# bmerry/mlsgpu

Measured on AMD Instinct MI355X. Metric: Mvoxels/s evaluated+triangulated, higher is better.
Workload: dtype f32; 1 GPU; cfg3: 512^3 grid, 50000000 splats (uniform), 27 buckets of <= 171 cells per side, octree+MLS+MC end-to-end; bucket_splats_total=52997386, mesh_memory_mb=4096, device_workers=3, batch=8, marching_group=2, mls_variant=culled+matrix-prefilter, counts_cover=the whole cloud

## Files before the change

mlsgpu_amd/csrc/api.hip:

```cpp
#include "common.hpp"

#include <algorithm>
#include <atomic>
#include <mutex>

using namespace mlsgpu;

namespace mlsgpu
{

static thread_local char lastError[512] = "";

int setError(int code, const char *fmt, ...)
{
    va_list ap;
    va_start(ap, fmt);
    vsnprintf(lastError, sizeof(lastError), fmt, ap);
    va_end(ap);
    return code;
}

}

MLSGPU_API const char *mlsgpu_hip_last_error(void) { return mlsgpu::lastError; }
// ... 170 lines not shown
        }
        ctx->ownStream = true;
    }
    *out = ctx;
    return MLSGPU_OK;
}

int mlsgpu_ctx::scanFlags(uint32_t **flags, uint32_t *epoch, uint32_t **tickets, uint32_t *bases, uint32_t gridX, uint32_t count)
{
    const size_t flagWords = (size_t) MLSGPU_MAX_BATCH * 1024;
    const size_t ticketWords = (size_t) MLSGPU_MAX_BATCH * 32;
    if (dScanFlags == nullptr)
    {
        HIP_CHECK(hipSetDevice(device));
        HIP_CHECK(hipMalloc((void **) &dScanFlags, (flagWords + ticketWords) * sizeof(uint32_t)));
        HIP_CHECK(hipMemsetAsync(dScanFlags, 0, (flagWords + ticketWords) * sizeof(uint32_t), stream));
    }
    if (++scanEpoch == 0)
    {
        HIP_CHECK(hipMemsetAsync(dScanFlags, 0, flagWords * sizeof(uint32_t), stream));
        scanEpoch = 1;
    }
    *flags = dScanFlags;
    *epoch = scanEpoch;
    *tickets = dScanFlags + flagWords;
    for (uint32_t k = 0; k < count; k++)
    {
        bases[k] = scanTicketBase[k];
        scanTicketBase[k] += gridX;
    }
    return MLSGPU_OK;
}

MLSGPU_API int mlsgpu_hip_ctx_release_scratch(mlsgpu_ctx *ctx)
{
    REQUIRE(ctx != nullptr, MLSGPU_ERR_INVALID);
    HIP_CHECK(hipSetDevice(ctx->device));
    HIP_CHECK(hipStreamSynchronize(ctx->stream));
    ctx->scratchCache.clear();
    return MLSGPU_OK;
}

MLSGPU_API void mlsgpu_hip_ctx_destroy(mlsgpu_ctx *ctx)
{
    if (!ctx)
        return;
    hipSetDevice(ctx->device);
    hipStreamSynchronize(ctx->stream);
    ctx->scratchCache.clear();
    hipFree(ctx->dScanFlags);
    for (const PendingTiming &p : ctx->pending)
    {
        hipEventDestroy(p.start);
        hipEventDestroy(p.stop);
    }
    for (hipEvent_t e : ctx->eventPool)
        hipEventDestroy(e);
    if (ctx->ownStream)
        hipStreamDestroy(ctx->stream);
    delete ctx;
}

MLSGPU_API void *mlsgpu_hip_ctx_stream(mlsgpu_ctx *ctx) { return ctx ? ctx->stream : nullptr; }

MLSGPU_API int mlsgpu_hip_ctx_synchronize(mlsgpu_ctx *ctx)
{
    REQUIRE(ctx != nullptr, MLSGPU_ERR_INVALID);
    HIP_CHECK(hipSetDevice(ctx->device));
    HIP_CHECK(hipStreamSynchronize(ctx->stream));
    return MLSGPU_OK;
}

MLSGPU_API int mlsgpu_hip_malloc(mlsgpu_ctx *ctx, size_t bytes, void **dptr)
{
    REQUIRE(ctx != nullptr && dptr != nullptr, MLSGPU_ERR_INVALID);
    HIP_CHECK(hipSetDevice(ctx->device));
    HIP_CHECK(hipMalloc(dptr, bytes ? bytes : 4));
    return MLSGPU_OK;
}

MLSGPU_API int mlsgpu_hip_free(mlsgpu_ctx *ctx, void *dptr)
{
    REQUIRE(ctx != nullptr, MLSGPU_ERR_INVALID);
// ... 427 lines not shown
```

mlsgpu_amd/csrc/common.hpp:

```cpp
#ifndef MLSGPU_AMD_COMMON_HPP
#define MLSGPU_AMD_COMMON_HPP

#include <hip/hip_runtime.h>

#include <cstdarg>
#include <cstdint>
#include <cstdio>
#include <cstring>
#include <map>
#include <memory>
#include <string>
#include <utility>
#include <vector>

#include "../../include/mlsgpu_hip.h"

#define MLSGPU_API extern "C" __attribute__((visibility("default")))

namespace mlsgpu
{


int setError(int code, const char *fmt, ...) __attribute__((format(printf, 2, 3)));

// ... 132 lines not shown

struct Stat
{
    double totalMs = 0.0;
    uint64_t launches = 0;
};

struct PendingTiming
{
    int nameId;
    hipEvent_t start, stop;
};

}

struct mlsgpu_ctx
{
    int device = 0;
    uint64_t serial = 0;
    hipStream_t stream = nullptr;
    bool ownStream = false;
    bool timing = false;
    std::vector<std::string> statNames;
    std::map<std::string, int> statIds;
    std::vector<mlsgpu::Stat> stats;
    std::vector<mlsgpu::PendingTiming> pending;
    std::vector<hipEvent_t> eventPool;
    std::map<std::string, std::shared_ptr<void> > scratchCache;

    uint32_t *dScanFlags = nullptr;
    uint32_t scanEpoch = 0;
    uint32_t scanTicketBase[MLSGPU_MAX_BATCH] = {};
    int scanFlags(uint32_t **flags, uint32_t *epoch, uint32_t **tickets, uint32_t *bases, uint32_t gridX, uint32_t count);

    int statId(const char *name);
    void addValue(const char *name, double value)
    {
        mlsgpu::Stat &st = stats[(size_t) statId(name)];
        st.totalMs += value;
        st.launches += 1;
    }
    int beginTiming(int id);
    void endTiming(int pendingIdx);
    int resolveTimings();
};

namespace mlsgpu
{

struct HostMailbox
{
    enum { WORDS = 64 };
    uint32_t *host = nullptr;
    uint32_t *dev = nullptr;
    uint32_t seq = 0;

    int create();
    void destroy();
    uint32_t reserve()
    {
        seq++;
        if (seq == 0)
            seq = 1;
        return seq;
    }
    int publish(hipStream_t stream, const void *src, uint32_t words);
// ... 121 lines not shown
```

mlsgpu_amd/csrc/mls.hip:

```cpp
#include "common.hpp"

#include <algorithm>
#include <cstdlib>

using namespace mlsgpu;

struct mlsgpu_tree;
extern "C" const mlsgpu_splat *mlsgpu_hip_tree_splats(const mlsgpu_tree *);
extern "C" const int32_t *mlsgpu_hip_tree_commands(const mlsgpu_tree *);
extern "C" const int32_t *mlsgpu_hip_tree_start(const mlsgpu_tree *);
extern "C" int mlsgpu_hip_tree_mutates(const mlsgpu_tree *);

struct mlsgpu_mls
{
    mlsgpu_ctx *ctx = nullptr;
    int shape = MLSGPU_SHAPE_SPHERE;
    int variant = 5;
    const mlsgpu_splat *dSplats = nullptr;
    const int32_t *dCommands = nullptr;
    const int32_t *dStart = nullptr;
    uint32_t startShift = 0;
    int32_t offset[3] = {0, 0, 0};
    float boundaryFactor = 0.0f;
    bool isSet = false;
// ... 178 lines not shown
    }
    return f;
}

__device__ __forceinline__ uint32_t spread3(uint32_t v)
{
    v &= 0x3FFu;
    v = (v | (v << 16)) & 0x030000FFu;
    v = (v | (v << 8)) & 0x0300F00Fu;
    v = (v | (v << 4)) & 0x030C30C3u;
    v = (v | (v << 2)) & 0x09249249u;
    return v;
}

struct MlsArgs
{
    float *field;
    uint64_t pitch;
    const float4 *splats;
    const int32_t *commands;
    const int32_t *start;
    uint32_t startShift;
    int32_t ox, oy, oz;
    uint32_t zStride;
    int32_t zBias;
    uint32_t zFirst;
    uint32_t blocksX, blocksY, blocksZ;
    uint32_t numBlocks;
    float boundaryFactor;
    uint32_t xcdChunk;
    uint32_t superShift, full, magicX, magicY;
    uint32_t rawRadius;
    unsigned long long *stats;
};

__device__ __forceinline__ float4 stagedPosRad(const MlsArgs &A, int32_t id)
{
    float4 pr = A.splats[2 * (int64_t) id];
    if (A.rawRadius)
        pr.w = 1.0f / (pr.w * pr.w);
    return pr;
}

__device__ __forceinline__ uint32_t xcdRemap(uint32_t id, uint32_t n, uint32_t chunk)
{
    if (chunk == 0)
    {
        const uint32_t q = n / 8, r = n % 8;
        const uint32_t xcd = id % 8, k = id / 8;
        return (xcd < r ? xcd * (q + 1) : r * (q + 1) + (xcd - r) * q) + k;
    }
    const uint32_t super = 8 * chunk;
    const uint32_t full = n / super * super;
    if (id >= full)
        return id;
    const uint32_t g = id / super, j = id % super;
    return g * super + (j % 8) * chunk + j / 8;
}

__device__ __forceinline__ int32_t listedId(const MlsArgs &A, int32_t pos, int32_t end, uint32_t slot)
{
    const int32_t lpos = pos + (int32_t) slot;
    return lpos < end ? A.commands[lpos] : -1;
}

struct ListRound
{
// ... 362 lines not shown
            __syncthreads();
        }
        fitUnpack(fit, sWpxy, sWnxy);
        f = finishCorner<SHAPE>(fit, A.boundaryFactor);
        if (STATS)
        {
            if (lane == 0)
                atomicAdd(&A.stats[5], (unsigned long long) sumMostPairs);
            addStats<true>(A, fit.hits, nListed, nTests, drainCalls, sumMost, sumMostRound, sHist);
        }
    }
    const int64_t row = (int64_t) (wy + ly) + (int64_t) (wz + lz) * A.zStride + A.zBias;
    A.field[row * (int64_t) A.pitch + (wx + lx)] = f;
}

typedef float f32x16 __attribute__((ext_vector_type(16)));
typedef __bf16 bf16x8 __attribute__((ext_vector_type(8)));

__device__ __forceinline__ void splitBf16(float x, uint32_t &hi, uint32_t &mid, uint32_t &lo)
{
    hi = __float_as_uint(x) & 0xFFFF0000u;
    const float r1 = x - __uint_as_float(hi);
    mid = __float_as_uint(r1) & 0xFFFF0000u;
    const float r2 = r1 - __uint_as_float(mid);
    lo = __float_as_uint(r2) & 0xFFFF0000u;
}

__device__ __forceinline__ uint32_t packHi(uint32_t e0, uint32_t e1)
{
    return __builtin_amdgcn_perm(e1, e0, 0x07060302u);
}

#define MATRIX_STAGE 512
#define MATRIX_SLOTS 440
#ifndef MLSGPU_MLS5_WAVES
#define MLSGPU_MLS5_WAVES 8
#endif


template<int SHAPE, bool STATS>
__global__ __launch_bounds__(512) __attribute__((amdgpu_waves_per_eu(MLSGPU_MLS5_WAVES, MLSGPU_MLS5_WAVES)))
void processCornersMatrixKernel(Lanes<MlsArgs> lanes)
{
    __shared__ float4 sPosRad[MATRIX_STAGE];
    __shared__ float4 sNormQ[MATRIX_STAGE];
    __shared__ uint4 sColLo[MATRIX_STAGE];
    __shared__ uint4 sColHi[MATRIX_STAGE];
    __shared__ alignas(8) uint8_t sMask[MATRIX_STAGE];
    __shared__ uint16_t sSlot[8][MATRIX_SLOTS + 40];
    __shared__ uint32_t sHist[STATS ? 33 : 1];
    static_assert(sizeof(sPosRad) + sizeof(sNormQ) + sizeof(sColLo) + sizeof(sColHi) + sizeof(sMask) + sizeof(sSlot) <= 40960,
                  "four workgroups per CU");

    const MlsArgs A = lanes.a[blockIdx.y];
    if (blockIdx.x >= A.numBlocks)
        return;
#ifdef MLSGPU_MLS5_CLOCK
    uint64_t clkMark = __builtin_amdgcn_s_memtime();
    const uint64_t clkStart = clkMark;
    uint64_t clkHead = 0, clkStage = 0, clkBar1 = 0, clkCompact = 0, clkTiles = 0, clkBar2 = 0;
#define MLS5_CLOCK(sum) do { uint64_t now_; asm volatile("s_memtime %0\n\ts_waitcnt lgkmcnt(0)" : "=s"(now_) : : "memory"); sum += now_ - clkMark; clkMark = now_; } while (0)
#else
#define MLS5_CLOCK(sum) do { } while (0)
#endif
    if (STATS)
    {
        if (threadIdx.x < 33)
            sHist[threadIdx.x] = 0;
        __syncthreads();
    }
    uint32_t gx, gy, gz;
    if (A.superShift != 0)
    {
        const uint32_t id = blockIdx.x, sh = A.superShift;
        const uint32_t j = id & ((1u << sh) - 1u);
        const uint32_t bid = id >= A.full ? id : (id >> sh << sh) + ((j & 7u) << (sh - 3u)) + (j >> 3);
        const uint32_t t = __umulhi(bid, A.magicX);
        gx = bid - t * A.blocksX;
        gz = __umulhi(t, A.magicY);
        gy = t - gz * A.blocksY;
    }
    else
    {
        const uint32_t bid = xcdRemap(blockIdx.x, A.numBlocks, A.xcdChunk);
        gx = bid % A.blocksX;
        gy = (bid / A.blocksX) % A.blocksY;
        gz = bid / (A.blocksX * A.blocksY);
    }
    const int wx = (int) (gx * 8), wy = (int) (gy * 8), wz = (int) (gz * 8 + A.zFirst);
    const uint32_t sub = A.startShift / 3;
    const uint32_t code = spread3((uint32_t) wx >> sub) | (spread3((uint32_t) wy >> sub) << 1) | (spread3((uint32_t) wz >> sub) << 2);
    int32_t pos = A.start[code];

    const uint32_t tid = threadIdx.x;
    const uint32_t wave = tid >> 6, lane = tid & 63;
    const int lx = (int) ((wave & 1) * 4 + (lane & 3));
    const int ly = (int) (((wave >> 1) & 1) * 4 + ((lane >> 2) & 3));
    const int lz = (int) ((wave >> 2) * 4 + (lane >> 4));

    float f = __int_as_float(0x7FC00000);
    if (pos >= 0)
    {
        const float cx = (float) (wx + lx + A.ox), cy = (float) (wy + ly + A.oy), cz = (float) (wz + lz + A.oz);

        float bx0, by0, bz0;
        float boxLo[3][2], boxHi[3][2];
        auto axisBounds = [](int o, float &lo0, float &hi0, float &lo1, float &hi1)
        {
            asm("s_nop 3\n\tv_readfirstlane_b32 %0, %4\n\tv_readfirstlane_b32 %1, %5\n\tv_readfirstlane_b32 %2, %6\n\t"
                "v_readfirstlane_b32 %3, %7\n\ts_nop 1"
                : "=s"(lo0), "=s"(hi0), "=s"(lo1), "=s"(hi1)
                : "v"((float) o), "v"((float) (o + 3)), "v"((float) (o + 4)), "v"((float) (o + 7)));
        };
        axisBounds(wx + A.ox, boxLo[0][0], boxHi[0][0], boxLo[0][1], boxHi[0][1]);
        axisBounds(wy + A.oy, boxLo[1][0], boxHi[1][0], boxLo[1][1], boxHi[1][1]);
        axisBounds(wz + A.oz, boxLo[2][0], boxHi[2][0], boxLo[2][1], boxHi[2][1]);
        bx0 = boxLo[0][0];
        by0 = boxLo[1][0];
        bz0 = boxLo[2][0];
        Fit fit;
        fitInit(fit);
        unsigned long long nListed = 0, nTests = 0, nCand = 0, nMissed = 0;
        uint32_t drainCalls = 0, sumMost = 0, sumMostRound = 0, roundCnt = 0;
        typedef __attribute__((address_space(3))) uint16_t LdsSlot;
        LdsSlot *const mySlots = (LdsSlot *) sSlot[wave] + 4;
        f32x2 sWpxy = {0.0f, 0.0f}, sWnxy = {0.0f, 0.0f};
        const f32x2 cxy = {cx, cy};

        uint4 bFrag[2];
        {
            const uint32_t n = lane & 31u, h = lane >> 5;
#pragma unroll
            for (uint32_t j = 0; j < 2; j++)
            {
                const uint32_t q = n + 32u * j;
                const uint32_t qx = (wave & 1u) * 4u + (q & 3u), qy = ((wave >> 1) & 1u) * 4u + ((q >> 2) & 3u), qz = (wave >> 2) * 4u + (q >> 4);
                const uint32_t u = h ? qz : qx, v = h ? qx * qx + qy * qy + qz * qz : qy;
                const uint32_t ub = __float_as_uint((float) u), vb = __float_as_uint((float) v);
                bFrag[j] = make_uint4(packHi(ub, ub), packHi(ub, vb), packHi(vb, vb), 0x3F803F80u);
            }
        }
        const uint32_t rowM = lane & 31u;
        const uint32_t rowSplat = 16u * ((rowM >> 2) & 1u) + 4u * (rowM >> 3) + (rowM & 3u);
        const char *const colBase = (lane >> 5) ? (const char *) sColHi : (const char *) sColLo;

        static_assert((MATRIX_SLOTS + 40) * sizeof(uint16_t) % 16 == 0 && (MATRIX_SLOTS + 40) * sizeof(uint16_t) <= 64 * 16, "one store per lane");
        if (lane < (MATRIX_SLOTS + 40) * sizeof(uint16_t) / 16)
            reinterpret_cast<uint4 *>(sSlot[wave])[lane] = make_uint4(0u, 0u, 0u, 0u);

        auto accumulate = [&](const float4 pr, const float4 nq)
        {
            const SplatOffset o = splatOffset(pr, cxy, cz);
            if (o.d < RADIUS_CUTOFF)
            {
                fitAddPacked(fit, sWpxy, sWnxy, o, nq);
                fit.hits++;
            }
        };
        auto ffbh = [](uint32_t v)
        {
            uint32_t t;
            asm("v_ffbh_u32 %0, %1" : "=v"(t) : "v"(v));
            return t;
        };
        auto posRadAt = [&](uint32_t off) { return *(const float4 *) ((const char *) sPosRad + off); };
        auto normQAt = [&](uint32_t off) { return *(const float4 *) ((const char *) sNormQ + off); };

        auto drain = [&](uint32_t cur, LdsSlot *chunk)
        {
            if (STATS)
            {
                const uint32_t cnt = (uint32_t) __popc(cur);
                drainCalls++;
                sumMost += waveMax(cnt);
                atomicAdd(&sHist[cnt], 1u);
                roundCnt += cnt;
                nCand += waveSum(cnt);
            }
            if (cur != 0)
            {
                uint32_t t = ffbh(cur);
                uint32_t off = chunk[t];
                float4 prA = posRadAt(off), nqA = normQAt(off), prB, nqB;
                for (;;)
                {
                    cur ^= 0x80000000u >> t;
                    t = ffbh(cur);
                    off = chunk[(int32_t) t];
                    prB = posRadAt(off);
                    nqB = normQAt(off);
                    accumulate(prA, nqA);
                    if (cur == 0)
                        break;
                    cur ^= 0x80000000u >> t;
                    t = ffbh(cur);
                    off = chunk[(int32_t) t];
                    prA = posRadAt(off);
                    nqA = normQAt(off);
                    accumulate(prB, nqB);
                    if (cur == 0)
                        break;
                }
            }
        };

        int32_t end = A.commands[pos++];
        int32_t idAhead = listedId(A, pos, end, tid);
        MLS5_CLOCK(clkHead);
        bool laterRound = false;
        while (pos < end)
        {
            {
                uint32_t mask = 0;
                const int32_t mine = idAhead;
                float4 pr = {0.0f, 0.0f, 0.0f, 0.0f}, nq = {0.0f, 0.0f, 0.0f, 0.0f};
                if (mine >= 0)
                {
                    pr = A.splats[2 * (int64_t) mine];
                    nq = A.splats[2 * (int64_t) mine + 1];
                }
                if (laterRound)
                {
                    asm volatile("s_waitcnt lgkmcnt(0)\n\ts_barrier" : : : "memory");
                    MLS5_CLOCK(clkBar2);
                }
                laterRound = true;
                if (mine >= 0)
                {
                    if (A.rawRadius)
                        pr.w = 1.0f / (pr.w * pr.w);
                    sPosRad[tid] = pr;
                    sNormQ[tid] = nq;
                    float d[3][2];
                    const float p[3] = {pr.x, pr.y, pr.z};
#pragma unroll
                    for (int a = 0; a < 3; a++)
#pragma unroll
                        for (int h = 0; h < 2; h++)
                            d[a][h] = fmaxf(fmaxf(boxLo[a][h] - p[a], p[a] - boxHi[a][h]), 0.0f);
#pragma unroll
                    for (int s_ = 7; s_ >= 0; s_--)
                    {
                        const float dx = d[0][s_ & 1], dy = d[1][(s_ >> 1) & 1], dz = d[2][s_ >> 2];
                        const float dd = dot3(dx, dy, dz, dx, dy, dz) * pr.w;
                        mask = __builtin_amdgcn_alignbit(mask, __float_as_uint(dd - RADIUS_CUTOFF), 31);
                    }
                    if (splatNeverCulled(pr))
                        mask = 0xFFu;
                    if (splatIsNan(pr))
                        mask = 0;

                    __builtin_amdgcn_sched_barrier(0);
                    const float ax = pr.x - bx0, ay = pr.y - by0, az = pr.z - bz0;
                    const float s1 = fabsf(ax) + fabsf(ay) + fabsf(az) + 21.0f;
                    const float T = fabsf(pr.w) * (s1 * s1);
                    const bool plain = T < 1e30f;
                    const float m2 = plain ? -2.0f * pr.w : 0.0f;
                    const float gc = plain ? fmaf(pr.w, dot3(ax, ay, az, ax, ay, az), -RADIUS_CUTOFF) - T * 0x1p-16f : -1.0f;
                    uint32_t c0, c1, c2;
                    splitBf16(gc, c0, c1, c2);
                    {
                        uint32_t x0, x1, x2, y0, y1, y2;
                        splitBf16(m2 * ax, x0, x1, x2);
                        splitBf16(m2 * ay, y0, y1, y2);
                        sColLo[tid] = make_uint4(packHi(x0, x1), packHi(x2, y0), packHi(y1, y2), packHi(c0, c1));
                    }
                    __builtin_amdgcn_sched_barrier(0);
                    {
                        uint32_t z0, z1, z2, q0, q1, q2;
                        splitBf16(m2 * az, z0, z1, z2);
                        splitBf16(plain ? pr.w : 0.0f, q0, q1, q2);
                        sColHi[tid] = make_uint4(packHi(z0, z1), packHi(z2, q0), packHi(q1, q2), c2 >> 16);
                    }
                }
                sMask[lane * 8 + wave] = (uint8_t) mask;
                if (STATS)
                    nListed += __popcll(__ballot(mine >= 0));
            }
            const ListRound r = listStep(A, pos, end, MATRIX_STAGE);
            pos = r.pos;
            end = r.end;
            const int32_t staged = r.staged;
            idAhead = listedId(A, pos, end, tid);
            MLS5_CLOCK(clkStage);
            __syncthreads();
            MLS5_CLOCK(clkBar1);

            int32_t g = 0;
            do
            {
            uint32_t nt = 0;
            const uint64_t mm = *(const uint64_t *) (sMask + lane * 8);
            for (; g < staged; g += 64)
            {
                const uint32_t m = (uint32_t) (mm >> ((uint32_t) g >> 3));
                const uint64_t todo = __ballot((m >> wave) & 1u);
                const uint32_t n = (uint32_t) __popcll(todo);
                if (nt + n > MATRIX_SLOTS)
                    break;
                if ((m >> wave) & 1u)
                    mySlots[nt + popcBelow(todo)] = (uint16_t) ((g + (int32_t) lane) * (int32_t) sizeof(float4));
                nt += n;
            }
            __builtin_amdgcn_fence(__ATOMIC_RELEASE, "wavefront");
            __builtin_amdgcn_wave_barrier();
            __builtin_amdgcn_fence(__ATOMIC_ACQUIRE, "wavefront");
            MLS5_CLOCK(clkCompact);
            __builtin_amdgcn_s_setprio(1);

            LdsSlot *tile = mySlots;
            for (uint32_t t0 = 0; t0 < nt; t0 += 32, tile += 32)
            {
                const uint32_t v = nt - t0 < 32u ? nt - t0 : 32u;
                const uint32_t off = tile[rowSplat];
                const uint4 aw = *(const uint4 *) (colBase + off);
                const bf16x8 aFrag = __builtin_bit_cast(bf16x8, aw);
                const f32x16 zero = {0.0f, 0.0f, 0.0f, 0.0f, 0.0f, 0.0f, 0.0f, 0.0f, 0.0f, 0.0f, 0.0f, 0.0f, 0.0f, 0.0f, 0.0f, 0.0f};
                uint32_t x0 = 0, x1 = 0;
                {
                    const f32x16 acc = __builtin_amdgcn_mfma_f32_32x32x16_bf16(aFrag, __builtin_bit_cast(bf16x8, bFrag[0]), zero, 0, 0, 0);
#pragma unroll
                    for (int r = 0; r < 16; r++)
                        x0 = __builtin_amdgcn_alignbit(x0, __float_as_uint(acc[r]), 31);
                }
                __builtin_amdgcn_sched_barrier(0);
                {
                    const f32x16 acc = __builtin_amdgcn_mfma_f32_32x32x16_bf16(aFrag, __builtin_bit_cast(bf16x8, bFrag[1]), zero, 0, 0, 0);
#pragma unroll
                    for (int r = 0; r < 16; r++)
                        x1 = __builtin_amdgcn_alignbit(x1, __float_as_uint(acc[r]), 31);
                }
                const auto sw = __builtin_amdgcn_permlane32_swap(x0, x1, false, false);
                uint32_t cur = (sw[0] << 16) | sw[1];
                cur &= 0xFFFFFFFFu << (32u - v);
                if (STATS)
                {
                    nTests += 64ull * 32ull;
                    uint32_t exact = 0;
                    for (uint32_t s = 0; s < v; s++)
                    {
                        const float d = splatOffset(posRadAt(tile[s]), cxy, cz).d;
                        exact |= d < RADIUS_CUTOFF ? 0x80000000u >> s : 0u;
                    }
                    nMissed += waveSum((uint32_t) __popc(exact & ~cur));
                }
#ifdef MLSGPU_MLS5_DUMP
                if (A.stats != nullptr && blockIdx.x % 499 == 0)
                {
                    unsigned long long at = 0;
                    if (lane == 0)
                        at = atomicAdd(&A.stats[0], 65ull);
                    at = __shfl(at, 0);
                    if (at + 65 < MLSGPU_MLS5_DUMP)
                    {
                        if (lane == 0)
                            A.stats[1 + at] = ((unsigned long long) blockIdx.y << 56) | ((unsigned long long) blockIdx.x << 24) | (wave << 16) | t0;
                        A.stats[2 + at + lane] = cur;
                    }
                }
#endif
                drain(cur, tile);
            }
            MLS5_CLOCK(clkTiles);
            } while (g < staged);
            __builtin_amdgcn_s_setprio(0);
            if (STATS)
            {
                sumMostRound += waveMax(roundCnt);
                roundCnt = 0;
            }
        }
        fitUnpack(fit, sWpxy, sWnxy);
        f = finishCorner<SHAPE>(fit, A.boundaryFactor);
#ifdef MLSGPU_MLS5_CLOCK
        if (A.stats != nullptr && lane == 0 && blockIdx.x % 61 == 0)
        {
            atomicAdd(&A.stats[0], (unsigned long long) clkHead);
            atomicAdd(&A.stats[1], (unsigned long long) clkStage);
            atomicAdd(&A.stats[2], (unsigned long long) clkBar1);
            atomicAdd(&A.stats[3], (unsigned long long) clkCompact);
            atomicAdd(&A.stats[4], (unsigned long long) clkTiles);
            atomicAdd(&A.stats[5], (unsigned long long) clkBar2);
            atomicAdd(&A.stats[6], (unsigned long long) (__builtin_amdgcn_s_memtime() - clkStart));
            atomicAdd(&A.stats[7], 1ull);
        }
#endif
        if (STATS)
        {
            if (lane == 0)
            {
                atomicAdd(&A.stats[41], nCand);
                atomicAdd(&A.stats[42], nMissed);
            }
            addStats<true>(A, fit.hits, nListed, nTests, drainCalls, sumMost, sumMostRound, sHist);
        }
    }
    const int64_t row = (int64_t) (wy + ly) + (int64_t) (wz + lz) * A.zStride + A.zBias;
    A.field[row * (int64_t) A.pitch + (wx + lx)] = f;
}

}


MLSGPU_API int mlsgpu_hip_mls_create(mlsgpu_ctx *ctx, int shape, mlsgpu_mls **out)
{
    REQUIRE(ctx != nullptr && out != nullptr, MLSGPU_ERR_INVALID);
    REQUIRE(shape == MLSGPU_SHAPE_SPHERE || shape == MLSGPU_SHAPE_PLANE, MLSGPU_ERR_INVALID);
    mlsgpu_mls *m = new mlsgpu_mls;
    m->ctx = ctx;
    m->shape = shape;
    *out = m;
    return mlsgpu_hip_mls_set_boundary_limit(m, 1.0f);
}

MLSGPU_API void mlsgpu_hip_mls_destroy(mlsgpu_mls *m) { delete m; }

MLSGPU_API int mlsgpu_hip_mls_set_buffers(mlsgpu_mls *m, const int32_t offset[3], const mlsgpu_splat *dSplats,
                                          const int32_t *dCommands, const int32_t *dStart, uint32_t subsamplingShift)
{
    REQUIRE(m != nullptr && offset != nullptr, MLSGPU_ERR_INVALID);
    REQUIRE(dSplats != nullptr && dCommands != nullptr && dStart != nullptr, MLSGPU_ERR_INVALID);
    REQUIRE(subsamplingShift >= 3 && subsamplingShift <= 10, MLSGPU_ERR_LENGTH);
    m->dSplats = dSplats;
    m->dCommands = dCommands;
    m->dStart = dStart;
    m->startShift = 3 * subsamplingShift;
    for (int i = 0; i < 3; i++)
        m->offset[i] = offset[i];
    m->isSet = true;
    m->rawRadius = false;
    return MLSGPU_OK;
// ... 8 lines not shown

MLSGPU_API int mlsgpu_hip_mls_set(mlsgpu_mls *m, const int32_t offset[3], const mlsgpu_tree *tree, uint32_t subsamplingShift)
{
    REQUIRE(m != nullptr && tree != nullptr, MLSGPU_ERR_INVALID);
    PROPAGATE(mlsgpu_hip_mls_set_buffers(m, offset, mlsgpu_hip_tree_splats(tree), mlsgpu_hip_tree_commands(tree),
                                         mlsgpu_hip_tree_start(tree), subsamplingShift));
    m->rawRadius = mlsgpu_hip_tree_mutates(tree) == 0;
    return MLSGPU_OK;
}

MLSGPU_API int mlsgpu_hip_mls_set_boundary_limit(mlsgpu_mls *m, float limit)
{
    REQUIRE(m != nullptr, MLSGPU_ERR_INVALID);
    const float pi = 3.14159265358979323846f;
    const float boundaryScale = (sqrtf(6.0f) * 512) / (693 * pi);
    const float gamma = boundaryScale * limit;
    m->boundaryFactor = 1.0f - gamma * gamma;
    return MLSGPU_OK;
}

MLSGPU_API int mlsgpu_hip_mls_set_variant(mlsgpu_mls *m, int variant)
{
    REQUIRE(m != nullptr && (variant == 1 || variant == 4 || variant == 5), MLSGPU_ERR_INVALID);
    m->variant = variant;
    return MLSGPU_OK;
}

MLSGPU_API int mlsgpu_hip_mls_set_stats(mlsgpu_mls *m, uint64_t *dCounters)
{
    REQUIRE(m != nullptr, MLSGPU_ERR_INVALID);
    m->dStats = reinterpret_cast<unsigned long long *>(dCounters);
    return MLSGPU_OK;
}

static int mlsLaneArgs(mlsgpu_mls *m, float *dField, uint64_t pitch, uint64_t fieldRows, const mlsgpu_swathe *sw, MlsArgs *out)
{
    REQUIRE(m != nullptr && dField != nullptr && sw != nullptr, MLSGPU_ERR_INVALID);
    REQUIRE(m->isSet, MLSGPU_ERR_INVALID);
    const uint32_t width = roundUp(sw->width, 8), height = roundUp(sw->height, 8);
    REQUIRE(sw->width > 0 && sw->height > 0, MLSGPU_ERR_INVALID);
    REQUIRE(sw->zStride >= height, MLSGPU_ERR_INVALID);
    REQUIRE(sw->zFirst <= sw->zLast, MLSGPU_ERR_INVALID);
    REQUIRE(sw->zFirst % 8 == 0, MLSGPU_ERR_INVALID);
    REQUIRE(pitch >= width, MLSGPU_ERR_LENGTH);
    const uint32_t blocksZ = divUp((uint64_t) sw->zLast - sw->zFirst + 1, 8);
    const int64_t firstRow = (int64_t) sw->zFirst * sw->zStride + sw->zBias;
    const int64_t lastRow = (int64_t) (sw->zFirst + 8 * blocksZ - 1) * sw->zStride + sw->zBias + height - 1;
    REQUIRE(firstRow >= 0 && (uint64_t) lastRow < fieldRows, MLSGPU_ERR_LENGTH);
    const uint32_t sub = m->startShift / 3;
    REQUIRE(((sw->zFirst + 8 * blocksZ - 1) >> sub) < 1024 && ((width - 1) >> sub) < 1024 && ((height - 1) >> sub) < 1024,
            MLSGPU_ERR_LENGTH);
    MlsArgs A;
    A.field = dField;
    A.pitch = pitch;
    A.splats = reinterpret_cast<const float4 *>(m->dSplats);
    A.commands = m->dCommands;
    A.start = m->dStart;
    A.startShift = m->startShift;
    A.ox = m->offset[0]; A.oy = m->offset[1]; A.oz = m->offset[2];
    A.zStride = sw->zStride;
    A.zBias = sw->zBias;
    A.zFirst = sw->zFirst;
    A.blocksX = width / 8;
    A.blocksY = height / 8;
    A.blocksZ = blocksZ;
    A.numBlocks = A.blocksX * A.blocksY * A.blocksZ;
    A.boundaryFactor = m->boundaryFactor;
    static const uint32_t xcdChunk = getenv("MLSGPU_HIP_MLS_XCD_CHUNK") ? (uint32_t) atoi(getenv("MLSGPU_HIP_MLS_XCD_CHUNK")) : 16u;
    A.xcdChunk = xcdChunk;
    A.superShift = A.full = A.magicX = A.magicY = 0;
    if (xcdChunk != 0 && (xcdChunk & (xcdChunk - 1)) == 0 && xcdChunk <= (1u << 20) && A.blocksX >= 2 && A.blocksY >= 2)
    {
        const uint64_t two32 = uint64_t(1) << 32;
        const uint64_t mx = (two32 + A.blocksX - 1) / A.blocksX, my = (two32 + A.blocksY - 1) / A.blocksY;
        const uint64_t nx = A.numBlocks - 1, ny = nx / A.blocksX;
        if (nx * (mx * A.blocksX - two32) < two32 && ny * (my * A.blocksY - two32) < two32)
        {
            uint32_t shift = 3;
            while ((1u << (shift - 3)) < xcdChunk)
                shift++;
            A.superShift = shift;
            A.full = A.numBlocks >> shift << shift;
            A.magicX = (uint32_t) mx;
            A.magicY = (uint32_t) my;
        }
    }
    A.rawRadius = m->rawRadius ? 1u : 0u;
    A.stats = m->dStats;
    *out = A;
    return MLSGPU_OK;
}

static int mlsEnqueueLanes(mlsgpu_mls *const *ms, const MlsArgs *args, uint32_t count)
{
    mlsgpu_mls *const m = ms[0];
    mlsgpu_ctx *ctx = m->ctx;
    for (uint32_t k = 1; k < count; k++)
        REQUIRE(ms[k]->ctx == ctx && ms[k]->shape == m->shape && ms[k]->variant == m->variant
                && (ms[k]->dStats != nullptr) == (m->dStats != nullptr), MLSGPU_ERR_INVALID);
    HIP_CHECK(hipSetDevice(ctx->device));
    const auto L = packLanes<MlsArgs>(count, [&](uint32_t k) { return args[k]; });
    const dim3 grid(mostOfLanes(count, [&](uint32_t k) { return args[k].numBlocks; }), count), block(512);
    const char *stat = "kernel.mls.processCorners.time";
    static const uint32_t ldsPad = [] {
        const char *e = getenv("MLSGPU_HIP_MLS_LDS_PAD");
        const long v = e ? atol(e) : 0;
        return (uint32_t) (v < 0 ? 0 : (v > 120 * 1024 ? 120 * 1024 : v));
    }();
#if defined(MLSGPU_MLS5_CLOCK) || defined(MLSGPU_MLS5_DUMP)
    const bool sphere = m->shape == MLSGPU_SHAPE_SPHERE, stats = m->dStats != nullptr && m->variant != 5;
#else
    const bool sphere = m->shape == MLSGPU_SHAPE_SPHERE, stats = m->dStats != nullptr;
#endif
#define MLS_LAUNCH(KERNEL, SHAPE, STATS) LAUNCH_LDS(ctx, stat, (KERNEL<SHAPE, STATS>), grid, block, ldsPad, L)
#define MLS_LAUNCH_ANY(KERNEL)                                                                                   \
    do {                                                                                                         \
        if (stats) { if (sphere) MLS_LAUNCH(KERNEL, MLSGPU_SHAPE_SPHERE, true); else MLS_LAUNCH(KERNEL, MLSGPU_SHAPE_PLANE, true); } \
        else { if (sphere) MLS_LAUNCH(KERNEL, MLSGPU_SHAPE_SPHERE, false); else MLS_LAUNCH(KERNEL, MLSGPU_SHAPE_PLANE, false); }     \
    } while (0)
    if (m->variant == 5)
        MLS_LAUNCH_ANY(processCornersMatrixKernel);
    else if (m->variant == 4)
        MLS_LAUNCH_ANY(processCornersCubeKernel);
    else
        MLS_LAUNCH_ANY(processCornersKernel);
#undef MLS_LAUNCH_ANY
#undef MLS_LAUNCH
    return MLSGPU_OK;
}

MLSGPU_API int mlsgpu_hip_mls_enqueue(mlsgpu_mls *m, float *dField, uint64_t pitch, uint64_t fieldRows,
                                      const mlsgpu_swathe *sw)
{
    MlsArgs A;
    PROPAGATE(mlsLaneArgs(m, dField, pitch, fieldRows, sw, &A));
// ... 92 lines not shown
```

Baseline: 9385 Mvoxels/s.

## Make MLS matrix kernel persistent with atomic per-XCD work queues and prefetch

Turns the MLS matrix kernel into a persistent kernel. A grid capped near resident occupancy pulls 8x8x8 blocks from eight per-XCD atomic queues in global memory. Wave 0 fetches the next block's coordinates and command range into double-buffered LDS during the first round of the current block, and the first listed ids are also fetched ahead. The aim is to cut per-workgroup launch and setup costs and tail imbalance, at the price of atomic contention and a queue reset done by the last exiting workgroup, which depends on every launched workgroup reaching that point.

```diff
diff --git a/mlsgpu_amd/csrc/api.hip b/mlsgpu_amd/csrc/api.hip
--- a/mlsgpu_amd/csrc/api.hip
+++ b/mlsgpu_amd/csrc/api.hip
@@ -226,6 +226,19 @@
     return MLSGPU_OK;
 }
 
+int mlsgpu_ctx::mlsQueues(uint32_t **queues)
+{
+    if (dMlsQueues == nullptr)
+    {
+        const size_t bytes = (size_t) MLSGPU_MAX_BATCH * MLS_QUEUE_WORDS * sizeof(uint32_t);
+        HIP_CHECK(hipSetDevice(device));
+        HIP_CHECK(hipMalloc((void **) &dMlsQueues, bytes));
+        HIP_CHECK(hipMemsetAsync(dMlsQueues, 0, bytes, stream));
+    }
+    *queues = dMlsQueues;
+    return MLSGPU_OK;
+}
+
 MLSGPU_API int mlsgpu_hip_ctx_release_scratch(mlsgpu_ctx *ctx)
 {
     REQUIRE(ctx != nullptr, MLSGPU_ERR_INVALID);
@@ -243,6 +256,7 @@
     hipStreamSynchronize(ctx->stream);
     ctx->scratchCache.clear();
     hipFree(ctx->dScanFlags);
+    hipFree(ctx->dMlsQueues);
     for (const PendingTiming &p : ctx->pending)
     {
         hipEventDestroy(p.start);
diff --git a/mlsgpu_amd/csrc/common.hpp b/mlsgpu_amd/csrc/common.hpp
--- a/mlsgpu_amd/csrc/common.hpp
+++ b/mlsgpu_amd/csrc/common.hpp
@@ -188,6 +188,10 @@
     uint32_t scanEpoch = 0;
     uint32_t scanTicketBase[MLSGPU_MAX_BATCH] = {};
     int scanFlags(uint32_t **flags, uint32_t *epoch, uint32_t **tickets, uint32_t *bases, uint32_t gridX, uint32_t count);
+
+    enum { MLS_QUEUE_WORDS = 32 };
+    uint32_t *dMlsQueues = nullptr;
+    int mlsQueues(uint32_t **queues);
 
     int statId(const char *name);
     void addValue(const char *name, double value)
diff --git a/mlsgpu_amd/csrc/mls.hip b/mlsgpu_amd/csrc/mls.hip
--- a/mlsgpu_amd/csrc/mls.hip
+++ b/mlsgpu_amd/csrc/mls.hip
@@ -234,7 +234,11 @@
     uint32_t superShift, full, magicX, magicY;
     uint32_t rawRadius;
     unsigned long long *stats;
+    uint32_t *queues;
+    uint32_t blocksPerWg;
 };
+
+enum { MLS_QUEUE_EXITS = 8 };
 
 __device__ __forceinline__ float4 stagedPosRad(const MlsArgs &A, int32_t id)
 {
@@ -663,14 +667,33 @@
 }
 
 #define MATRIX_STAGE 512
-#define MATRIX_SLOTS 440
+#define MATRIX_SLOTS 432
 #ifndef MLSGPU_MLS5_WAVES
 #define MLSGPU_MLS5_WAVES 8
 #endif
 
+__device__ __forceinline__ uint32_t ldsUniform(const uint32_t *p)
+{
+    return (uint32_t) __builtin_amdgcn_readfirstlane((int) *p);
+}
+
+__device__ __forceinline__ float uniformFloat(int v)
+{
+    return __uint_as_float((uint32_t) __builtin_amdgcn_readfirstlane((int) __builtin_amdgcn_mbcnt_lo(0u, __float_as_uint((float) v))));
+}
+
+__device__ __forceinline__ uint32_t freshLaneId()
+{
+    uint32_t zero;
+    asm volatile("s_mov_b32 %0, 0" : "=s"(zero));
+    return __builtin_amdgcn_mbcnt_hi(~0u, __builtin_amdgcn_mbcnt_lo(~0u, zero));
+}
+
+enum { NEXT_GX = 0, NEXT_GY, NEXT_GZ, NEXT_POS, NEXT_END, NEXT_WORDS = 8 };
+#define NEXT_NONE 0xFFFFFFFFu
 
 template<int SHAPE, bool STATS>
-__global__ __launch_bounds__(512) __attribute__((amdgpu_waves_per_eu(MLSGPU_MLS5_WAVES, MLSGPU_MLS5_WAVES)))
+__global__ __launch_bounds__(512) __attribute__((amdgpu_waves_per_eu(STATS ? 6 : MLSGPU_MLS5_WAVES, STATS ? 6 : MLSGPU_MLS5_WAVES)))
 void processCornersMatrixKernel(Lanes<MlsArgs> lanes)
 {
     __shared__ float4 sPosRad[MATRIX_STAGE];
@@ -679,17 +702,17 @@
     __shared__ uint4 sColHi[MATRIX_STAGE];
     __shared__ alignas(8) uint8_t sMask[MATRIX_STAGE];
     __shared__ uint16_t sSlot[8][MATRIX_SLOTS + 40];
+    __shared__ alignas(16) uint32_t sNext[2][NEXT_WORDS];
     __shared__ uint32_t sHist[STATS ? 33 : 1];
-    static_assert(sizeof(sPosRad) + sizeof(sNormQ) + sizeof(sColLo) + sizeof(sColHi) + sizeof(sMask) + sizeof(sSlot) <= 40960,
-                  "four workgroups per CU");
+    static_assert(sizeof(sPosRad) + sizeof(sNormQ) + sizeof(sColLo) + sizeof(sColHi) + sizeof(sMask) + sizeof(sSlot) + sizeof(sNext)
+                  <= 40960, "four workgroups per CU");
 
     const MlsArgs A = lanes.a[blockIdx.y];
-    if (blockIdx.x >= A.numBlocks)
-        return;
 #ifdef MLSGPU_MLS5_CLOCK
     uint64_t clkMark = __builtin_amdgcn_s_memtime();
     const uint64_t clkStart = clkMark;
-    uint64_t clkHead = 0, clkStage = 0, clkBar1 = 0, clkCompact = 0, clkTiles = 0, clkBar2 = 0;
+    uint64_t clkHead = 0, clkStage = 0, clkBar1 = 0, clkCompact = 0, clkTiles = 0, clkBar2 = 0, clkBetween = 0;
+    uint32_t clkBlocks = 0;
 #define MLS5_CLOCK(sum) do { uint64_t now_; asm volatile("s_memtime %0\n\ts_waitcnt lgkmcnt(0)" : "=s"(now_) : : "memory"); sum += now_ - clkMark; clkMark = now_; } while (0)
 #else
 #define MLS5_CLOCK(sum) do { } while (0)
@@ -698,147 +721,220 @@
     {
         if (threadIdx.x < 33)
             sHist[threadIdx.x] = 0;
-        __syncthreads();
-    }
-    uint32_t gx, gy, gz;
-    if (A.superShift != 0)
-    {
-        const uint32_t id = blockIdx.x, sh = A.superShift;
-        const uint32_t j = id & ((1u << sh) - 1u);
-        const uint32_t bid = id >= A.full ? id : (id >> sh << sh) + ((j & 7u) << (sh - 3u)) + (j >> 3);
-        const uint32_t t = __umulhi(bid, A.magicX);
-        gx = bid - t * A.blocksX;
-        gz = __umulhi(t, A.magicY);
-        gy = t - gz * A.blocksY;
-    }
-    else
-    {
-        const uint32_t bid = xcdRemap(blockIdx.x, A.numBlocks, A.xcdChunk);
-        gx = bid % A.blocksX;
-        gy = (bid / A.blocksX) % A.blocksY;
-        gz = bid / (A.blocksX * A.blocksY);
-    }
-    const int wx = (int) (gx * 8), wy = (int) (gy * 8), wz = (int) (gz * 8 + A.zFirst);
-    const uint32_t sub = A.startShift / 3;
-    const uint32_t code = spread3((uint32_t) wx >> sub) | (spread3((uint32_t) wy >> sub) << 1) | (spread3((uint32_t) wz >> sub) << 2);
-    int32_t pos = A.start[code];
-
-    const uint32_t tid = threadIdx.x;
-    const uint32_t wave = tid >> 6, lane = tid & 63;
+    }
+
+    const uint32_t wave = (uint32_t) __builtin_amdgcn_readfirstlane((int) (threadIdx.x >> 6)), lane = laneId();
+    const uint32_t tid = wave * 64u + lane;
     const int lx = (int) ((wave & 1) * 4 + (lane & 3));
     const int ly = (int) (((wave >> 1) & 1) * 4 + ((lane >> 2) & 3));
     const int lz = (int) ((wave >> 2) * 4 + (lane >> 4));
-
-    float f = __int_as_float(0x7FC00000);
-    if (pos >= 0)
-    {
-        const float cx = (float) (wx + lx + A.ox), cy = (float) (wy + ly + A.oy), cz = (float) (wz + lz + A.oz);
-
-        float bx0, by0, bz0;
+    const bool fetcher = wave == 0;
+
+    typedef __attribute__((address_space(3))) uint16_t LdsSlot;
+    LdsSlot *const mySlots = (LdsSlot *) sSlot[wave] + 4;
+
+    uint4 bFrag[2];
+    {
+        const uint32_t n = lane & 31u, h = lane >> 5;
+#pragma unroll
+        for (uint32_t j = 0; j < 2; j++)
+        {
+            const uint32_t q = n + 32u * j;
+            const uint32_t qx = (wave & 1u) * 4u + (q & 3u), qy = ((wave >> 1) & 1u) * 4u + ((q >> 2) & 3u), qz = (wave >> 2) * 4u + (q >> 4);
+            const uint32_t u = h ? qz : qx, v = h ? qx * qx + qy * qy + qz * qz : qy;
+            const uint32_t ub = __float_as_uint((float) u), vb = __float_as_uint((float) v);
+            bFrag[j] = make_uint4(packHi(ub, ub), packHi(ub, vb), packHi(vb, vb), 0x3F803F80u);
+        }
+    }
+    const uint32_t rowM = lane & 31u;
+    const uint32_t rowSplat = 16u * ((rowM >> 2) & 1u) + 4u * (rowM >> 3) + (rowM & 3u);
+    const char *const colBase = (lane >> 5) ? (const char *) sColHi : (const char *) sColLo;
+
+    static_assert((MATRIX_SLOTS + 40) * sizeof(uint16_t) % 16 == 0 && (MATRIX_SLOTS + 40) * sizeof(uint16_t) <= 64 * 16, "one store per lane");
+    if (lane < (MATRIX_SLOTS + 40) * sizeof(uint16_t) / 16)
+        reinterpret_cast<uint4 *>(sSlot[wave])[lane] = make_uint4(0u, 0u, 0u, 0u);
+
+    uint32_t queue = __builtin_amdgcn_s_getreg(20 | (3 << 11)) & 7u;
+    uint32_t drawn = 0;
+    auto fetchNext = [&](uint32_t slot)
+    {
+        typedef const __attribute__((address_space(4))) MlsArgs *KernelArgs;
+        KernelArgs R = (KernelArgs) __builtin_amdgcn_kernarg_segment_ptr() + blockIdx.y;
+        asm volatile("" : "+s"(R));
+        uint32_t id = NEXT_NONE;
+        if (drawn < R->blocksPerWg)
+        {
+#pragma unroll 1
+            for (uint32_t tries = 0; tries < 8u; tries++)
+            {
+                uint32_t n = 0;
+                if (lane == 0)
+                    n = __hip_atomic_fetch_add(&R->queues[queue], 1u, __ATOMIC_RELAXED, __HIP_MEMORY_SCOPE_AGENT);
+                n = (uint32_t) __builtin_amdgcn_readfirstlane((int) n);
+                if (n < (R->numBlocks + 7u - queue) / 8u)
+                {
+                    id = 8u * n + queue;
+                    break;
+                }
+                queue = (queue + 1u) & 7u;
+            }
+            drawn++;
+        }
+        uint32_t gx = NEXT_NONE, gy = 0, gz = 0;
+        int32_t pos = -1, end = 0;
+        if (id != NEXT_NONE)
+        {
+            if (R->superShift != 0)
+            {
+                const uint32_t sh = R->superShift;
+                const uint32_t j = id & ((1u << sh) - 1u);
+                const uint32_t bid = id >= R->full ? id : (id >> sh << sh) + ((j & 7u) << (sh - 3u)) + (j >> 3);
+                const uint32_t t = __umulhi(bid, R->magicX);
+                gx = bid - t * R->blocksX;
+                gz = __umulhi(t, R->magicY);
+                gy = t - gz * R->blocksY;
+            }
+            else
+            {
+                const uint32_t bid = xcdRemap(id, R->numBlocks, R->xcdChunk);
+                gx = bid % R->blocksX;
+                gy = (bid / R->blocksX) % R->blocksY;
+                gz = bid / (R->blocksX * R->blocksY);
+            }
+            const uint32_t sub = R->startShift / 3;
+            const uint32_t code = spread3((gx * 8u) >> sub) | (spread3((gy * 8u) >> sub) << 1) | (spread3((gz * 8u + R->zFirst) >> sub) << 2);
+            pos = R->start[code];
+            if (pos >= 0)
+                end = R->commands[pos];
+        }
+        if (lane == 0)
+        {
+            *reinterpret_cast<uint4 *>(sNext[slot]) = make_uint4(gx, gy, gz, (uint32_t) pos);
+            sNext[slot][NEXT_END] = (uint32_t) end;
+        }
+    };
+
+    Fit fit;
+    float f;
+    f32x2 sWpxy, sWnxy;
+    f32x2 cxy;
+    float cz;
+    unsigned long long nListed = 0, nTests = 0, nCand = 0, nMissed = 0, hitTotal = 0;
+    uint32_t drainCalls = 0, sumMost = 0, sumMostRound = 0, sumMostBlock = 0, roundCnt = 0;
+
+    auto accumulate = [&](const float4 pr, const float4 nq)
+    {
+        const SplatOffset o = splatOffset(pr, cxy, cz);
+        if (o.d < RADIUS_CUTOFF)
+        {
+            fitAddPacked(fit, sWpxy, sWnxy, o, nq);
+            fit.hits++;
+        }
+    };
+    auto ffbh = [](uint32_t v)
+    {
+        uint32_t t;
+        asm("v_ffbh_u32 %0, %1" : "=v"(t) : "v"(v));
+        return t;
+    };
+    auto posRadAt = [&](uint32_t off) { return *(const float4 *) ((const char *) sPosRad + off); };
+    auto normQAt = [&](uint32_t off) { return *(const float4 *) ((const char *) sNormQ + off); };
+
+    auto drain = [&](uint32_t cur, LdsSlot *chunk)
+    {
+        if (STATS)
+        {
+            const uint32_t cnt = (uint32_t) __popc(cur);
+            drainCalls++;
+            sumMost += waveMax(cnt);
+            atomicAdd(&sHist[cnt], 1u);
+            roundCnt += cnt;
+            nCand += waveSum(cnt);
+        }
+        if (cur != 0)
+        {
+            uint32_t t = ffbh(cur);
+            uint32_t off = chunk[t];
+            float4 prA = posRadAt(off), nqA = normQAt(off), prB, nqB;
+            for (;;)
+            {
+                cur ^= 0x80000000u >> t;
+                t = ffbh(cur);
+                off = chunk[(int32_t) t];
+                prB = posRadAt(off);
+                nqB = normQAt(off);
+                accumulate(prA, nqA);
+                if (cur == 0)
+                    break;
+                cur ^= 0x80000000u >> t;
+                t = ffbh(cur);
+                off = chunk[(int32_t) t];
+                prA = posRadAt(off);
+                nqA = normQAt(off);
+                accumulate(prB, nqB);
+                if (cur == 0)
+                    break;
+            }
+        }
+    };
+
+    bool laterRound = false;
+    bool haveIds = false;
+    int32_t idAhead = -1;
+    for (uint32_t blk = 0;; blk++)
+    {
+        const uint32_t *const now = sNext[blk & 1u];
+        uint32_t gx = 0, gy = 0, gz = 0;
+        int32_t pos = -1;
+        if (blk != 0)
+        {
+            gx = ldsUniform(now + NEXT_GX);
+            if (gx == NEXT_NONE)
+                break;
+            gy = ldsUniform(now + NEXT_GY);
+            gz = ldsUniform(now + NEXT_GZ);
+            pos = (int32_t) ldsUniform(now + NEXT_POS);
+        }
+        const int wx = (int) (gx * 8), wy = (int) (gy * 8), wz = (int) (gz * 8 + A.zFirst);
+        auto store = [&](float v)
+        {
+            const int64_t row = (int64_t) (wy + ly) + (int64_t) (wz + lz) * A.zStride + A.zBias;
+            A.field[row * (int64_t) A.pitch + (wx + lx)] = v;
+        };
+        if (pos < 0)
+        {
+            if (blk != 0)
+                store(__int_as_float(0x7FC00000));
+            if (fetcher)
+                fetchNext((blk + 1u) & 1u);
+            __syncthreads();
+            haveIds = false;
+            continue;
+        }
+        int32_t end = (int32_t) ldsUniform(now + NEXT_END);
+        pos++;
+        cxy = f32x2{(float) (wx + lx + A.ox), (float) (wy + ly + A.oy)};
+        cz = (float) (wz + lz + A.oz);
         float boxLo[3][2], boxHi[3][2];
-        auto axisBounds = [](int o, float &lo0, float &hi0, float &lo1, float &hi1)
-        {
-            asm("s_nop 3\n\tv_readfirstlane_b32 %0, %4\n\tv_readfirstlane_b32 %1, %5\n\tv_readfirstlane_b32 %2, %6\n\t"
-                "v_readfirstlane_b32 %3, %7\n\ts_nop 1"
-                : "=s"(lo0), "=s"(hi0), "=s"(lo1), "=s"(hi1)
-                : "v"((float) o), "v"((float) (o + 3)), "v"((float) (o + 4)), "v"((float) (o + 7)));
-        };
-        axisBounds(wx + A.ox, boxLo[0][0], boxHi[0][0], boxLo[0][1], boxHi[0][1]);
-        axisBounds(wy + A.oy, boxLo[1][0], boxHi[1][0], boxLo[1][1], boxHi[1][1]);
-        axisBounds(wz + A.oz, boxLo[2][0], boxHi[2][0], boxLo[2][1], boxHi[2][1]);
-        bx0 = boxLo[0][0];
-        by0 = boxLo[1][0];
-        bz0 = boxLo[2][0];
-        Fit fit;
+        {
+            const int o[3] = {wx + A.ox, wy + A.oy, wz + A.oz};
+#pragma unroll
+            for (int a = 0; a < 3; a++)
+            {
+                boxLo[a][0] = uniformFloat(o[a]);
+                boxHi[a][0] = uniformFloat(o[a] + 3);
+                boxLo[a][1] = uniformFloat(o[a] + 4);
+                boxHi[a][1] = uniformFloat(o[a] + 7);
+            }
+        }
+        const float bx0 = boxLo[0][0], by0 = boxLo[1][0], bz0 = boxLo[2][0];
         fitInit(fit);
-        unsigned long long nListed = 0, nTests = 0, nCand = 0, nMissed = 0;
-        uint32_t drainCalls = 0, sumMost = 0, sumMostRound = 0, roundCnt = 0;
-        typedef __attribute__((address_space(3))) uint16_t LdsSlot;
-        LdsSlot *const mySlots = (LdsSlot *) sSlot[wave] + 4;
-        f32x2 sWpxy = {0.0f, 0.0f}, sWnxy = {0.0f, 0.0f};
-        const f32x2 cxy = {cx, cy};
-
-        uint4 bFrag[2];
-        {
-            const uint32_t n = lane & 31u, h = lane >> 5;
-#pragma unroll
-            for (uint32_t j = 0; j < 2; j++)
-            {
-                const uint32_t q = n + 32u * j;
-                const uint32_t qx = (wave & 1u) * 4u + (q & 3u), qy = ((wave >> 1) & 1u) * 4u + ((q >> 2) & 3u), qz = (wave >> 2) * 4u + (q >> 4);
-                const uint32_t u = h ? qz : qx, v = h ? qx * qx + qy * qy + qz * qz : qy;
-                const uint32_t ub = __float_as_uint((float) u), vb = __float_as_uint((float) v);
-                bFrag[j] = make_uint4(packHi(ub, ub), packHi(ub, vb), packHi(vb, vb), 0x3F803F80u);
-            }
-        }
-        const uint32_t rowM = lane & 31u;
-        const uint32_t rowSplat = 16u * ((rowM >> 2) & 1u) + 4u * (rowM >> 3) + (rowM & 3u);
-        const char *const colBase = (lane >> 5) ? (const char *) sColHi : (const char *) sColLo;
-
-        static_assert((MATRIX_SLOTS + 40) * sizeof(uint16_t) % 16 == 0 && (MATRIX_SLOTS + 40) * sizeof(uint16_t) <= 64 * 16, "one store per lane");
-        if (lane < (MATRIX_SLOTS + 40) * sizeof(uint16_t) / 16)
-            reinterpret_cast<uint4 *>(sSlot[wave])[lane] = make_uint4(0u, 0u, 0u, 0u);
-
-        auto accumulate = [&](const float4 pr, const float4 nq)
-        {
-            const SplatOffset o = splatOffset(pr, cxy, cz);
-            if (o.d < RADIUS_CUTOFF)
-            {
-                fitAddPacked(fit, sWpxy, sWnxy, o, nq);
-                fit.hits++;
-            }
-        };
-        auto ffbh = [](uint32_t v)
-        {
-            uint32_t t;
-            asm("v_ffbh_u32 %0, %1" : "=v"(t) : "v"(v));
-            return t;
-        };
-        auto posRadAt = [&](uint32_t off) { return *(const float4 *) ((const char *) sPosRad + off); };
-        auto normQAt = [&](uint32_t off) { return *(const float4 *) ((const char *) sNormQ + off); };
-
-        auto drain = [&](uint32_t cur, LdsSlot *chunk)
-        {
-            if (STATS)
-            {
-                const uint32_t cnt = (uint32_t) __popc(cur);
-                drainCalls++;
-                sumMost += waveMax(cnt);
-                atomicAdd(&sHist[cnt], 1u);
-                roundCnt += cnt;
-                nCand += waveSum(cnt);
-            }
-            if (cur != 0)
-            {
-                uint32_t t = ffbh(cur);
-                uint32_t off = chunk[t];
-                float4 prA = posRadAt(off), nqA = normQAt(off), prB, nqB;
-                for (;;)
-                {
-                    cur ^= 0x80000000u >> t;
-                    t = ffbh(cur);
-                    off = chunk[(int32_t) t];
-                    prB = posRadAt(off);
-                    nqB = normQAt(off);
-                    accumulate(prA, nqA);
-                    if (cur == 0)
-                        break;
-                    cur ^= 0x80000000u >> t;
-                    t = ffbh(cur);
-                    off = chunk[(int32_t) t];
-                    prA = posRadAt(off);
-                    nqA = normQAt(off);
-                    accumulate(prB, nqB);
-                    if (cur == 0)
-                        break;
-                }
-            }
-        };
-
-        int32_t end = A.commands[pos++];
-        int32_t idAhead = listedId(A, pos, end, tid);
+        sWpxy = f32x2{0.0f, 0.0f};
+        sWnxy = f32x2{0.0f, 0.0f};
+        if (!haveIds)
+            idAhead = listedId(A, pos, end, wave * 64u + freshLaneId());
         MLS5_CLOCK(clkHead);
-        bool laterRound = false;
+        bool firstRound = true;
         while (pos < end)
         {
             {
@@ -856,6 +952,9 @@
                     MLS5_CLOCK(clkBar2);
                 }
                 laterRound = true;
+                if (firstRound && fetcher)
+                    fetchNext((blk + 1u) & 1u);
+                firstRound = false;
                 if (mine >= 0)
                 {
                     if (A.rawRadius)
@@ -912,10 +1011,30 @@
             pos = r.pos;
             end = r.end;
             const int32_t staged = r.staged;
-            idAhead = listedId(A, pos, end, tid);
+            const bool lastRound = !(pos < end);
+            if (!lastRound)
+                idAhead = listedId(A, pos, end, wave * 64u + freshLaneId());
             MLS5_CLOCK(clkStage);
             __syncthreads();
             MLS5_CLOCK(clkBar1);
+            if (lastRound)
+            {
+                const uint32_t *const next = sNext[(blk + 1u) & 1u];
+                const int32_t npos = (int32_t) ldsUniform(next + NEXT_POS);
+                haveIds = npos >= 0;
+                idAhead = haveIds ? listedId(A, npos + 1, (int32_t) ldsUniform(next + NEXT_END), wave * 64u + freshLaneId()) : -1;
+            }
+
+            if (STATS)
+            {
+                for (int32_t s = 0; s < staged; s++)
+                {
+                    const uint32_t m = sMask[(s & 63) * 8 + (s >> 6)];
+                    const float d = splatOffset(sPosRad[s], cxy, cz).d;
+                    const bool missed = ((m >> wave) & 1u) == 0 && d < RADIUS_CUTOFF;
+                    nMissed += (unsigned long long) __popcll(__ballot(missed));
+                }
+            }
 
             int32_t g = 0;
             do
@@ -976,7 +1095,7 @@
                     nMissed += waveSum((uint32_t) __popc(exact & ~cur));
                 }
 #ifdef MLSGPU_MLS5_DUMP
-                if (A.stats != nullptr && blockIdx.x % 499 == 0)
+                if (A.stats != nullptr && blockIdx.x % 31 == 0)
                 {
                     unsigned long long at = 0;
                     if (lane == 0)
@@ -1003,31 +1122,59 @@
         }
         fitUnpack(fit, sWpxy, sWnxy);
         f = finishCorner<SHAPE>(fit, A.boundaryFactor);
+        store(f);
+        if (STATS)
+        {
+            hitTotal += waveSum(fit.hits);
+            sumMostBlock += waveMax(fit.hits);
+        }
 #ifdef MLSGPU_MLS5_CLOCK
-        if (A.stats != nullptr && lane == 0 && blockIdx.x % 61 == 0)
-        {
-            atomicAdd(&A.stats[0], (unsigned long long) clkHead);
-            atomicAdd(&A.stats[1], (unsigned long long) clkStage);
-            atomicAdd(&A.stats[2], (unsigned long long) clkBar1);
-            atomicAdd(&A.stats[3], (unsigned long long) clkCompact);
-            atomicAdd(&A.stats[4], (unsigned long long) clkTiles);
-            atomicAdd(&A.stats[5], (unsigned long long) clkBar2);
-            atomicAdd(&A.stats[6], (unsigned long long) (__builtin_amdgcn_s_memtime() - clkStart));
-            atomicAdd(&A.stats[7], 1ull);
-        }
+        clkBlocks++;
 #endif
-        if (STATS)
-        {
-            if (lane == 0)
-            {
-                atomicAdd(&A.stats[41], nCand);
-                atomicAdd(&A.stats[42], nMissed);
-            }
-            addStats<true>(A, fit.hits, nListed, nTests, drainCalls, sumMost, sumMostRound, sHist);
-        }
-    }
-    const int64_t row = (int64_t) (wy + ly) + (int64_t) (wz + lz) * A.zStride + A.zBias;
-    A.field[row * (int64_t) A.pitch + (wx + lx)] = f;
+        MLS5_CLOCK(clkBetween);
+    }
+
+#ifdef MLSGPU_MLS5_CLOCK
+    if (A.stats != nullptr && lane == 0 && blockIdx.x % 7 == 0)
+    {
+        atomicAdd(&A.stats[0], (unsigned long long) clkHead);
+        atomicAdd(&A.stats[1], (unsigned long long) clkStage);
+        atomicAdd(&A.stats[2], (unsigned long long) clkBar1);
+        atomicAdd(&A.stats[3], (unsigned long long) clkCompact);
+        atomicAdd(&A.stats[4], (unsigned long long) clkTiles);
+        atomicAdd(&A.stats[5], (unsigned long long) clkBar2);
+        atomicAdd(&A.stats[6], (unsigned long long) clkBetween);
+        atomicAdd(&A.stats[7], (unsigned long long) (__builtin_amdgcn_s_memtime() - clkStart));
+        atomicAdd(&A.stats[8], 1ull);
+        atomicAdd(&A.stats[9], (unsigned long long) clkBlocks);
+    }
+#endif
+    if (STATS)
+    {
+        if (lane == 0)
+        {
+            atomicAdd(&A.stats[0], nListed);
+            atomicAdd(&A.stats[1], nTests);
+            atomicAdd(&A.stats[2], hitTotal);
+            atomicAdd(&A.stats[3], (unsigned long long) drainCalls);
+            atomicAdd(&A.stats[4], (unsigned long long) sumMost);
+            atomicAdd(&A.stats[6], (unsigned long long) sumMostRound);
+            atomicAdd(&A.stats[7], (unsigned long long) sumMostBlock);
+            atomicAdd(&A.stats[41], nCand);
+            atomicAdd(&A.stats[42], nMissed);
+        }
+        __syncthreads();
+        if (threadIdx.x < 33 && sHist[threadIdx.x] != 0)
+            atomicAdd(&A.stats[8 + threadIdx.x], (unsigned long long) sHist[threadIdx.x]);
+    }
+
+    if (threadIdx.x == 0)
+    {
+        const uint32_t left = __hip_atomic_fetch_add(&A.queues[MLS_QUEUE_EXITS], 1u, __ATOMIC_RELAXED, __HIP_MEMORY_SCOPE_AGENT);
+        if (left + 1u == gridDim.x)
+            for (uint32_t k = 0; k <= MLS_QUEUE_EXITS; k++)
+                __hip_atomic_store(&A.queues[k], 0u, __ATOMIC_RELAXED, __HIP_MEMORY_SCOPE_AGENT);
+    }
 }
 
 }
@@ -1102,6 +1249,10 @@
     m->dStats = reinterpret_cast<unsigned long long *>(dCounters);
     return MLSGPU_OK;
 }
+
+#ifndef MLS_BLOCKS_PER_WG
+#define MLS_BLOCKS_PER_WG 8
+#endif
 
 static int mlsLaneArgs(mlsgpu_mls *m, float *dField, uint64_t pitch, uint64_t fieldRows, const mlsgpu_swathe *sw, MlsArgs *out)
 {
@@ -1157,11 +1308,13 @@
     }
     A.rawRadius = m->rawRadius ? 1u : 0u;
     A.stats = m->dStats;
+    A.queues = nullptr;
+    A.blocksPerWg = 1;
     *out = A;
     return MLSGPU_OK;
 }
 
-static int mlsEnqueueLanes(mlsgpu_mls *const *ms, const MlsArgs *args, uint32_t count)
+static int mlsEnqueueLanes(mlsgpu_mls *const *ms, MlsArgs *args, uint32_t count)
 {
     mlsgpu_mls *const m = ms[0];
     mlsgpu_ctx *ctx = m->ctx;
@@ -1169,8 +1322,27 @@
         REQUIRE(ms[k]->ctx == ctx && ms[k]->shape == m->shape && ms[k]->variant == m->variant
                 && (ms[k]->dStats != nullptr) == (m->dStats != nullptr), MLSGPU_ERR_INVALID);
     HIP_CHECK(hipSetDevice(ctx->device));
+    uint32_t gridX = mostOfLanes(count, [&](uint32_t k) { return args[k].numBlocks; });
+    if (m->variant == 5)
+    {
+        int cus = 0;
+        const uint32_t resident = hipDeviceGetAttribute(&cus, hipDeviceAttributeMultiprocessorCount, ctx->device) == hipSuccess && cus > 0
+                                      ? 4u * (uint32_t) cus : 1024u;
+        const char *const kEnv = getenv("MLSGPU_HIP_MLS_BLOCKS_PER_WG"), *const wgEnv = getenv("MLSGPU_HIP_MLS_WORKGROUPS");
+        const long perWg = kEnv ? atol(kEnv) : MLS_BLOCKS_PER_WG, wgs = wgEnv ? atol(wgEnv) : (long) (resident / count);
+        const uint32_t blocksPerWg = (uint32_t) std::min<long>(std::max<long>(perWg, 1), 1l << 30);
+        const uint32_t cap = (uint32_t) std::min<long>(std::max<long>(wgs, 1), 1l << 30);
+        gridX = std::min(divUp(gridX, blocksPerWg), cap);
+        uint32_t *queues = nullptr;
+        PROPAGATE(ctx->mlsQueues(&queues));
+        for (uint32_t k = 0; k < count; k++)
+        {
+            args[k].queues = queues + (size_t) k * mlsgpu_ctx::MLS_QUEUE_WORDS;
+            args[k].blocksPerWg = std::max(blocksPerWg, divUp(args[k].numBlocks, gridX));
+        }
+    }
     const auto L = packLanes<MlsArgs>(count, [&](uint32_t k) { return args[k]; });
-    const dim3 grid(mostOfLanes(count, [&](uint32_t k) { return args[k].numBlocks; }), count), block(512);
+    const dim3 grid(gridX, count), block(512);
     const char *stat = "kernel.mls.processCorners.time";
     static const uint32_t ldsPad = [] {
         const char *e = getenv("MLSGPU_HIP_MLS_LDS_PAD");
```

Result: slower. 8882 Mvoxels/s (-5.4%).
